# mrazomej/BarBay.jl

Measured on AMD Instinct MI355X. Metric: ELBO-grad steps/sec, 50k barcodes x 8 timepoints, higher is better.
Workload: dtype f64

## Files before the change

### barbay.jl_amd/csrc/bb_engine.hip

```cpp
#include "../../include/barbay_hip.h"
#include "bb_block.h"
#include "bb_persist.h"
#include "bb_resident.h"
#include "bb_stream.h"
#include "bb_inst.h"
#include "bb_hier.h"
#include "bb_ppc.h"

#include <algorithm>
#include <cmath>
#include <cstdarg>
#include <cstdio>
#include <cstdlib>
#include <cstring>
#include <ctime>
#include <string>
#include <type_traits>
#include <vector>

#ifndef BB_EMU
#include <dlfcn.h>
#endif

static thread_local char g_err[512] = "";
// ... 147 lines not shown
    const char* names[] = {"librccl.so.1", "librccl.so", "/opt/rocm/lib/librccl.so.1"};
    for (const char* n : names) {
        g_rccl.lib = dlopen(n, RTLD_NOW | RTLD_GLOBAL);
        if (g_rccl.lib) break;
    }
    if (!g_rccl.lib) return bb_fail(BB_ERR_COMM, "cannot load librccl: %s", dlerror());
    g_rccl.GetUniqueId = (int (*)(bb_ncclUniqueId*))dlsym(g_rccl.lib, "ncclGetUniqueId");
    g_rccl.CommInitRank = (int (*)(bb_ncclComm_t*, int, bb_ncclUniqueId, int))dlsym(g_rccl.lib, "ncclCommInitRank");
    g_rccl.AllReduce = (int (*)(const void*, void*, size_t, int, int, bb_ncclComm_t, hipStream_t))dlsym(g_rccl.lib, "ncclAllReduce");
    g_rccl.CommDestroy = (int (*)(bb_ncclComm_t))dlsym(g_rccl.lib, "ncclCommDestroy");
    g_rccl.GetErrorString = (const char* (*)(int))dlsym(g_rccl.lib, "ncclGetErrorString");
    if (!g_rccl.GetUniqueId || !g_rccl.CommInitRank || !g_rccl.AllReduce || !g_rccl.CommDestroy)
        return bb_fail(BB_ERR_COMM, "librccl lacks a required symbol");
    return 0;
}
#endif

#ifdef BB_EMU
struct DevGuard { explicit DevGuard(int) {} };
#else
struct DevGuard {
    int prev = -1, dev;
    explicit DevGuard(int d) : dev(d) { if (hipGetDevice(&prev) != hipSuccess) prev = -1; if (prev != dev) (void)hipSetDevice(dev); }
    ~DevGuard() { if (prev >= 0 && prev != dev) (void)hipSetDevice(prev); }
    DevGuard(const DevGuard&) = delete;
    DevGuard& operator=(const DevGuard&) = delete;
};
#endif
#define BB_ENTER(h) DevGuard bb_dev_guard_((h)->o.device)

struct BBTuning {
    bool no_hist_pack, no_host_tables, no_res, no_persist, no_stream, force_stream, any_parity, force_allreduce, p2p_self;
    bool no_graph, graph_collective, no_regroup, no_reorder, nb_set, lead_set;
    int nb, res_nb, ng, lead, nthr, row_l2;
};

static BBTuning read_tuning() {
    auto set = [](const char* n) { return getenv(n) != nullptr; };
    auto num = [](const char* n, int unset) { const char* v = getenv(n); return v ? atoi(v) : unset; };
    auto on = [&](const char* n) { return num(n, 0) > 0; };
    BBTuning t{};
    t.no_hist_pack = on("BB_NO_HIST_PACK");
    t.no_host_tables = on("BB_NO_HOST_TABLES");
    t.no_res = on("BB_NO_RES");
    t.no_persist = on("BB_NO_PERSIST");
    t.no_stream = on("BB_NO_STREAM");
    t.force_stream = on("BB_TUNE_STREAM");
    t.any_parity = on("BB_TUNE_AP");
    t.force_allreduce = on("BB_FORCE_ALLREDUCE");
    t.p2p_self = on("BB_P2P_SELF");
    t.no_graph = set("BB_NO_GRAPH");
    t.graph_collective = set("BB_GRAPH_COLLECTIVE");
    t.no_regroup = set("BB_NO_REGROUP");
    t.no_reorder = set("BB_NO_REORDER");
    t.nb_set = set("BB_TUNE_NB");
    t.nb = num("BB_TUNE_NB", 0);
    t.res_nb = num("BB_TUNE_RES_NB", 0);
    t.ng = num("BB_TUNE_NG", 0);
    t.lead_set = set("BB_TUNE_LEAD");
    t.lead = num("BB_TUNE_LEAD", 65);
    if (t.lead < 10 || t.lead > 100) t.lead = 100;
    t.nthr = num("BB_TUNE_NTHR", 0) >= 64 ? num("BB_TUNE_NTHR", 0) / 64 * 64 : 0;
    t.row_l2 = num("BB_TUNE_ROW_L2", 1) == 0 ? 0 : 1;
    return t;
}

enum { IMPL_TWO_KERNEL = 0, IMPL_PERSIST = 1, IMPL_RES = 2, IMPL_STREAM = 3 };
struct LaunchPlan {
    int impl = IMPL_TWO_KERNEL;
    int P = 0;
    int NB = 0, NBL = 0, nblk = 0;
    int ng = 8, pf = 0;
    bool ms = false;
    const void* fn = nullptr;
    std::string name;
    const char* why = nullptr;
};

struct bb_handle {
    DevModel M{};
    DevState S{};
    bb_advi_opts o{};
    std::vector<bb_block_range> blocks;
    std::vector<void*> owned;
    long long dev_bytes = 0;
    int NB = 0, nthr = 0, nblk = 0, ngeno_blk = 0;
    int tile_cap = 0;
    size_t lds_doubles = 0;
    size_t lds_doubles_p0 = 0;
    size_t lds_doubles_p = 0;
    long long b_lo = 0, b_hi = 0;
    int cus = 256;
    int g_lo = 0, g_hi = 0;
    std::vector<int> geno_ptr_h;
    long long* d_tile_b = nullptr;
// ... 561 lines not shown
    bb_handle* h = E.h;
    const RunArgs& A = E.A;
    BRSt<PP>* st = (BRSt<PP>*)E.st.data();
    auto cxof = [&](int b) { return BBCtx{h->nthr, b, E.lds.data() + (size_t)b * (h->lds_doubles_p + 64), nullptr}; };
    const BRLay& Y = h->Yh;
    const int NS = A.S < 1 ? 1 : A.S;
    const bool MSrun = NS > 1 || A.elbo_every > 0;
    const unsigned long long step = (unsigned long long)(h->step + it / NS);
    const int smp = (int)(it % NS);
    const bool last = smp == NS - 1;
    const unsigned long long xc = MSrun ? step * (unsigned long long)NS + (unsigned long long)smp : step;
    const int buf = (int)(xc & 1);
    const bool want_el = MSrun && A.elbo_every > 0 && step % (unsigned long long)A.elbo_every == 0;
    const int ring = A.elbo_every > 0 ? (int)((step / (unsigned long long)A.elbo_every) % BB_ELBO_RING) : 0;
    const bool xg = h->p2p_on;
    const BBSlot wslot = bb_slot_of(A, step);
    for (int b = 0; b < (phase == 2 ? bbp_groups(A) : h->plan.nblk); ++b) {
        BBCtx cx = cxof(b);
        BRSt<PP>* sb = st + (size_t)b * h->nthr;
        if (phase == 0) {
            br_prologue<KIND, PP, AP>(cx, h->M, h->S, A, Y, h->plan.NB, sb);
            br_draw_ahead<KIND, PP, AP>(cx, A, Y, sb, (unsigned long long)h->step);
        } else if (phase == 1) {
            if (MSrun) br_sample<KIND, PP, true>(cx, h->M, h->S, A, Y, sb, buf, wslot.slot, last, want_el);
            else br_sample<KIND, PP, false>(cx, h->M, h->S, A, Y, sb, buf, wslot.slot);
            const unsigned epoch = A.xepoch0 + (unsigned)(xc + 1);
            if (MSrun) br_moments<KIND, PP, true>(cx, h->M, h->S, Y, sb, buf, epoch, want_el);
            else br_moments<KIND, PP, false>(cx, h->M, h->S, Y, sb, buf, epoch);
            br_xchg_publish<KIND, PP, AP>(cx, h->M, h->S, A, Y, sb, xc, wslot.slot, last ? step + 1 : step, last ? 0u : (unsigned)(smp + 1), last);
        } else if (phase == 2) {
            if (xg) br_xchg_lead<true>(cx, h->M, h->S, A, Y, xc, &E.ok);
            else br_xchg_lead<false>(cx, h->M, h->S, A, Y, xc, &E.ok);
        } else if (phase == 3) {
            if (xg && MSrun) br_xchg_consume<KIND, PP, true, true>(cx, h->M, h->S, A, Y, sb, xc, &E.ok, want_el, ring, smp);
            else if (xg) br_xchg_consume<KIND, PP, true, false>(cx, h->M, h->S, A, Y, sb, xc, &E.ok);
            else if (MSrun) br_xchg_consume<KIND, PP, false, true>(cx, h->M, h->S, A, Y, sb, xc, &E.ok, want_el, ring, smp);
            else br_xchg_consume<KIND, PP, false, false>(cx, h->M, h->S, A, Y, sb, xc, &E.ok);
            if (MSrun) br_update<KIND, PP, 0, AP, true>(cx, h->M, h->S, A, Y, sb, wslot, buf, h->plan.NB, smp, NS);
            else if (!AP && uniform_T(h->M) == 8) br_update<KIND, PP, 8, false>(cx, h->M, h->S, A, Y, sb, wslot, buf, h->plan.NB);
            else if (!AP && uniform_T(h->M) == 6) br_update<KIND, PP, 6, false>(cx, h->M, h->S, A, Y, sb, wslot, buf, h->plan.NB);
            else br_update<KIND, PP, 0, AP>(cx, h->M, h->S, A, Y, sb, wslot, buf, h->plan.NB);
        } else {
            br_epilogue<KIND, PP, AP>(cx, h->S, sb, (unsigned long long)(h->step + nsteps), E.ok == 0);
        }
    }
}

template <int KIND, int TT, bool MS>
static void emu_stream_phase(EmuPersist& E, int phase, long long it, long long nsteps) {
    bb_handle* h = E.h;
    const RunArgs& A = E.A;
    BSG* gs = (BSG*)E.st.data();
    auto cxof = [&](int b) { return BBCtx{h->nthr, b, E.lds.data() + (size_t)b * (h->lds_doubles_p + 64), nullptr}; };
    const BRLay& Y = h->Yh;
    const int NS = MS ? (A.S < 1 ? 1 : A.S) : 1;
    const unsigned long long step = (unsigned long long)(h->step + it / NS);
    const int smp = (int)(it % NS);
    const unsigned long long xc = step * (unsigned long long)NS + (unsigned long long)smp;
    auto rec = [&](unsigned long long st_) { return MS && A.elbo_every > 0 && st_ % (unsigned long long)A.elbo_every == 0; };
    const bool want_el = rec(step);
    const int ring = A.elbo_every > 0 ? (int)((step / (unsigned long long)A.elbo_every) % BB_ELBO_RING) : 0;
    const BSMs ms = MS ? bs_ms_of(A, step, smp, NS, want_el, rec(step + 1)) : bs_ms_plain((unsigned)step);
    BRSt<1>* nost = nullptr;
    for (int b = 0; b < (phase == 2 ? bbp_groups(A) : h->plan.nblk); ++b) {
        BBCtx cx = cxof(b);
        BSG* gb = gs + (size_t)b * h->nthr;
        int* bad_any = (int*)(cx.lds + Y.L.misc) + 3;
        if (phase == 0) {
            br_tile_setup<KIND>(cx, h->M, h->S, A, Y, h->plan.NB, KIND <= 2 ? h->nthr / 16 : h->nthr / 64);
            *bad_any = 0;
// ... 577 lines not shown
    free(h->hstatus);
#else
    if (h->hstatus) (void)hipHostFree(h->hstatus);
#endif
    for (void* p : h->owned) dfree(p);
    if (h->eps_buf) dfree(h->eps_buf);
    if (h->dbg_buf) dfree(h->dbg_buf);
    if (h->ppc_buf) dfree(h->ppc_buf);
#ifndef BB_EMU
    if (h->stream) (void)hipStreamDestroy(h->stream);
#endif
    delete h;
}

extern "C" int64_t bb_num_latents(const bb_handle* h) { return h ? h->M.D : 0; }

extern "C" int bb_get_layout(const bb_handle* h, bb_block_range* blocks, int32_t* n) {
    if (!h || !blocks || !n) return bb_fail(BB_ERR_INVALID, "null argument");
    *n = (int32_t)h->blocks.size();
    for (size_t i = 0; i < h->blocks.size(); ++i) blocks[i] = h->blocks[i];
    return BB_OK;
}

static RunArgs make_args(const bb_handle* h, long long step, int sample, int S, bool apply, bool with_elbo) {
    RunArgs A;
    memset(&A, 0, sizeof A);
    A.b_lo = h->b_lo;
    A.b_hi = h->b_hi;
    A.rank = h->o.rank;
    A.world = h->o.world_size;
    A.xepoch0 = h->epoch0;
    A.spin_limit = 1u << 23;
    A.row_l2 = h->tune.row_l2;
    A.nblk = h->nblk;
    A.nblk_alloc = h->tile_cap - 8;
    A.ng = 8;
    A.par = (int)(step & 1);
    A.sample = sample;
    A.S = S;
    A.first_sample = sample == 0;
    A.last_sample = sample == S - 1;
    A.apply = apply ? 1 : 0;
    A.with_elbo = with_elbo ? 1 : 0;
    A.count_globals = h->o.rank == 0;
    A.opt = h->o.optimizer;
    A.W = h->o.window;
    A.resum_every = h->o.resum_every;
    A.elbo_every = h->o.elbo_every;
    A.eta = h->o.eta;
    A.tau = h->o.tau;
    A.pre = h->o.pre;
    A.post = h->o.post;
    A.seed = h->o.seed;
    A.elbo_const = h->elbo_const;
    if (h->use_reduce()) { A.red = h->S.totals; A.nred = 1; }
    else { A.red = h->S.partials; A.nred = h->nblk; }
    return A;
}

#ifdef BB_EMU
#define LAUNCH_CHECK() 0
#else
static int launch_check() {
    hipError_t e = hipGetLastError();
    if (e != hipSuccess) return bb_fail(BB_ERR_DEVICE, "kernel launch: %s", hipGetErrorString(e));
    return 0;
// ... 1257 lines not shown
```

### barbay.jl_amd/csrc/bb_persist.h

```cpp
#pragma once
#include "bb_block.h"
#include <string.h>

template <int KIND>
BB_DEV BBLds bbp_layout(const BBCtx& cx, const DevModel& M, int NB) {
    if (cx.lay) return *(const BBLds*)cx.lay;
    return bb_lds_layout(M.R, M.E, KIND, M.Ttot, M.nt1, M.K, NB, cx.nthr, 1);
}

template <int P>
struct BBPst {
    bb_d2 mu[P], om[P], am[P], ao[P];
    bb_d2 a[P], h[P];
    bb_d2 hm[P], ho[P];
    long long i0[P];
    int meta[P];
    bb_f4 lo[P];
};

#ifdef BB_EMU
#define BB_PSTATE(stv, tid) ((stv)[tid])
#else
#define BB_PSTATE(stv, tid) ((stv)[0])
#endif
// ... 398 lines not shown
        BB_SYNC(cx);
        BB_PASS(cx, tid) {
            if (tid < KK) {
                double s = lds[L.red + tid];
                for (int c = 1; c < chunks; ++c) s += lds[L.red + c * KKP + tid];
                if (XG) { for (int r = 0; r < A.world; ++r) bb_gran_st<true>(S.xgr[r] + bbx_slot(A, par, A.rank, g) * KK + tid, s, epoch); }
                else bb_gran_st(S.gxrow + ((long long)par * NG + g) * KK + tid, s, epoch);
            }
        }
        BB_SYNC(cx);
        BB_STAMP(cx, S, 18);
        return;
    }
    BB_PASS(cx, tid) {
        if (tid < KKP) {
            const bool act = tid < KK;
            const int k = act ? tid : KK - 1;
            double s = 0.0;
            for (int m0 = 0; m0 < members; m0 += 8) {
                double v[8];
                const int n = members - m0 < 8 ? members - m0 : 8;
                if (!bb_gran_poll8(S.grow + (long long)g * KS, (unsigned)(m0 * NG * KS + k), (unsigned)(NG * KS), n, epoch, act, S.gbar + 1, A.spin_limit, v)) *ok = 0;
#pragma unroll
                for (int i = 0; i < 8; ++i) s += v[i];
            }
            if (XG) {
                if (act) for (int r = 0; r < A.world; ++r) bb_gran_st<true>(S.xgr[r] + bbx_slot(A, par, A.rank, g) * KK + k, s, epoch);
            } else if (act) bb_gran_st(S.gxrow + ((long long)par * NG + g) * KK + k, s, epoch);
        }
    }
    BB_STAMP(cx, S, 18);
}

BB_DEV void bbp_consume_tg(BBCtx& cx, const DevModel& M, const DevState& S, const RunArgs& A, const BBLds& L, int par, unsigned epoch, int* ok) {
    double* lds = cx.lds;
    const int KK = M.K + 2 * M.nt1, NG = bbp_groups(A);
    const int KKP = (KK + 63) & ~63, NQ = (NG + 7) >> 3;
    double s0 = 0.0;
    BB_PASS(cx, tid) {
        const int q = (tid >= KKP ? 1 : 0) + (tid >= 2 * KKP ? 1 : 0) + (tid >= 3 * KKP ? 1 : 0) + (tid >= 4 * KKP ? 1 : 0), kk = tid - q * KKP;
        if (q < NQ) {
            const bool act = kk < KK;
            const int k = act ? kk : KK - 1, g0 = 8 * q;
            double v[8];
            const int n = NG - g0 < 8 ? NG - g0 : 8;
            if (!bb_gran_poll8(S.gxrow + (long long)par * NG * KK, (unsigned)(g0 * KK + k), (unsigned)KK, n, epoch, act, S.gbar + 1, A.spin_limit, v)) *ok = 0;
            double s = 0.0;
#pragma unroll
            for (int i = 0; i < 8; ++i) s += v[i];
            if (q > 0) { if (act) lds[L.red + (q - 1) * KKP + kk] = s; }
            else {
#ifdef BB_EMU
                if (act) lds[L.red + 3 * KKP + kk] = s;
#else
                s0 = s;
#endif
            }
        }
    }
    BB_STAMP(cx, S, 1);
    BB_SYNC(cx);
    BB_PASS(cx, tid) {
        if (tid < KK) {
#ifdef BB_EMU
            s0 = lds[L.red + 3 * KKP + tid];
#endif
            double s = s0;
            for (int q = 1; q < NQ; ++q) s += lds[L.red + (q - 1) * KKP + tid];
            if (tid < M.K) bb_put_total(M, L, lds, tid, s);
            else lds[L.zgl + (tid - M.K)] = s;
        }
    }
    if (!(KK <= 64 && M.Ttot <= 64)) BB_SYNC(cx);
}

BB_DEV void bbp_consume_tgx(BBCtx& cx, const DevModel& M, const DevState& S, const RunArgs& A, const BBLds& L, int par, unsigned epoch, int* ok) {
    double* lds = cx.lds;
    const int KK = M.K + 2 * M.nt1, KKP = (KK + 63) & ~63, chunks = A.world;
    int NQ = cx.nthr / KKP;
    if (NQ > chunks) NQ = chunks;
    if (NQ < 1) NQ = 1;
    const bb_gran* in = S.xgr[A.rank] + (long long)par * A.world * 8 * KK;
    BB_PASS(cx, tid) {
        int q = 0;
        for (int t = KKP; t <= tid && q < NQ; t += KKP) ++q;
        const int kk = tid - q * KKP;
        if (q < NQ) {
            const bool act = kk < KK;
            const int k = act ? kk : KK - 1;
            for (int c = q; c < chunks; c += NQ) {
                double v[8];
                if (!bb_gran_poll8<true>(in, (unsigned)(c * 8 * KK + k), (unsigned)KK, 8, epoch, act, S.gbar + 1, A.spin_limit, v)) *ok = 0;
                double s = 0.0;
#pragma unroll
// ... 313 lines not shown
```

### barbay.jl_amd/csrc/bb_resident.h

```cpp
#pragma once
#include "bb_persist.h"

#define BR_NCV 12
#if defined(BB_EMU) || defined(BR_NO_FENCE)
#define BR_SCHED_FENCE() ((void)0)
#else
#define BR_SCHED_FENCE() __builtin_amdgcn_sched_barrier(0)
#endif
#define BR_MAXT 16

struct BRSeg { long long lo, hi; int tbeg, span, blk, kind, ldsoff, r, lpb, T; double pm, iv; const double* mean_e; const double* iv_e; long long blo; int rstride, pad; };
#define BR_SEG_DOUBLES 12

struct BRLay {
    BBLds L;
    int zl, NBT;
    int zr0[BB_MAX_REP];
    int zlw, stw;
    int st[6], SU, nst;
    int eps;
    int hbuf;
    int racc;
    int racc_r[BB_MAX_REP], rw[BB_MAX_REP];
    int rowmap;
// ... 124 lines not shown
        Y.hbuf = o;    o += 4 * P * NT;
    } else {
        Y.hbuf = Y.racc;
        Y.eps = Y.hbuf + 4 * P * NT;
        busy = 6 * P * NT;
        o += racc_total > busy ? racc_total : busy;
    }
    { const int nch = xg_rows / 8 > 5 ? xg_rows / 8 : 5;
      L.red = o;     o += 2 * 128 + nch * ((KK + 63) & ~63) + 16; }
    (void)lmax;
    L.total = Y.total = (o + 1) & ~1;
    return Y;
}

template <int P>
struct BRSt {
    bb_d2 mu[P], om[P], am[P], ao[P];
    bb_d2 a[P], h[P];
    bb_d2 z[P];
    bb_d2 lam[P];
    long long i0[P];
    int meta[P];
    int zoff[P];
    int uo[P][3];
    int pt[P];
    int rb[P];
    int thoff[P];
    unsigned cnt[P][2];
    bb_f4 lo[P];
    bb_d2 gp[P];
    bb_d2 gm[P], go[P];
    double el;
};

enum { BRM_A0 = 1 << 4, BRM_A1 = 1 << 5, BRM_VALID = 1 << 6, BRM_MUT = 1 << 7, BRM_PREV = 1 << 8, BRM_NEXT = 1 << 9 };

template <bool AP> BB_DEV bool br_pair_aligned(long long i0) { return !AP || !(i0 & 1); }
template <bool AP> BB_DEV bb_d2 br_load_pair(const double* base, long long i0, bool a0, bool a1) {
    if (a0 && a1 && br_pair_aligned<AP>(i0)) return *(const bb_d2*)(base + i0);
    return bb_d2{a0 ? base[i0] : 0.0, a1 ? base[i0 + 1] : 0.0};
}
template <bool AP> BB_DEV void br_store_pair_stream(double* base, long long i0, bool a0, bool a1, bb_d2 v) {
#ifndef BB_EMU
    if (a0 && a1 && br_pair_aligned<AP>(i0)) {
        typedef double bb_v2d __attribute__((ext_vector_type(2)));
        bb_v2d w = {v.x, v.y};
        __builtin_nontemporal_store(w, (bb_v2d*)(base + i0));
        return;
    }
    if (a0) __builtin_nontemporal_store(v.x, base + i0);
    if (a1) __builtin_nontemporal_store(v.y, base + i0 + 1);
#else
    if (a0 && a1 && br_pair_aligned<AP>(i0)) { *(bb_d2*)(base + i0) = v; return; }
    if (a0) base[i0] = v.x;
    if (a1) base[i0 + 1] = v.y;
#endif
}
template <bool AP> BB_DEV void br_store_pair(double* base, long long i0, bool a0, bool a1, bb_d2 v) {
    if (a0 && a1 && br_pair_aligned<AP>(i0)) { *(bb_d2*)(base + i0) = v; return; }
    if (a0) base[i0] = v.x;
    if (a1) base[i0 + 1] = v.y;
}

BB_HD BBTile br_tile(const DevModel& M, const RunArgs& A, int block, int NB) {
    if (A.nbl <= 0) return bb_tile(M, A, block, NB);
    const int nlead = bbp_groups(A);
// ... 152 lines not shown
    st.meta[k] = meta;
}

BB_HD void br_table_row(const DevModel& M, const BRLay& Y, int j, int* rm2, int* tmapj) {
    int code = 0, col = 0;
    for (int r = 0; r < M.R; ++r) {
        const int T = M.T[r], q0 = j - M.kq[r];
        if (q0 < 0 || q0 >= 6 * T - 5) continue;
        int tt, q;
        if (q0 < T) { tt = q0; q = 0; } else { tt = (q0 - T) / 5; q = 1 + (q0 - T) - 5 * tt; }
        code = Y.lpb[r] | (1 << 24);
        col = Y.racc_r[r] + ((tt & 1) * 6 + q) * (Y.rw[r] + 4) + (tt >> 1);
    }
    rm2[0] = code;
    rm2[1] = col;
    int tj = -1;
    for (int r = 0; r < M.R; ++r) { const int tt = j - M.kq[r]; if (tt >= 0 && tt < M.T[r]) tj = M.tcum[r] + tt; }
    *tmapj = tj;
}
BB_HD void br_table_time(const DevModel& M, const BBLds& L, int j, int* ft) {
    int r = 0;
    while (r + 1 < M.R && j >= M.tcum[r + 1]) ++r;
    const int tt = j - M.tcum[r], T = M.T[r];
    ft[0] = tt < T - 1 ? L.wk + M.kq[r] + T + 5 * tt : -1;
    ft[1] = M.off_t[r] + tt;
    ft[2] = tt > 0 ? 1 : 0;
    ft[3] = 0;
}
BB_HD void br_table_rep(const DevModel& M, const BRLay& Y, int r, int* rt) {
    rt[0] = M.tcum[r]; rt[1] = Y.zr0[r]; rt[2] = M.T[r];
    rt[3] = M.cnt_off[r] < (1ll << 31) ? (int)M.cnt_off[r] : -1;
}

template <int KIND>
BB_DEV void br_tile_setup(BBCtx& cx, const DevModel& M, const DevState& S, const RunArgs& A, const BRLay& Y, int NB, int ncol_or_neg) {
    double* lds = cx.lds;
    const BBLds& L = Y.L;
    const BBTile t = KIND == 2 ? br_tile_geno(M, S, cx.block, NB) : br_tile(M, A, cx.block, NB);
    const int g0 = KIND == 2 ? S.tile_g[cx.block] : 0, g1 = KIND == 2 ? S.tile_g[cx.block + 1] : 0;
    BRSeg* sg = (BRSeg*)(lds + Y.seg);
    int* li = (int*)(lds + L.misc);
    const int KK = M.K + 2 * M.nt1;
    BB_PASS(cx, tid) {
        if (S.segtab) {
            const double* src = S.segtab + (long long)cx.block * S.segtab_stride;
            const int nd = S.segtab_stride - 1;
            for (int i = tid; i < nd; i += cx.nthr) lds[Y.seg + i] = src[i];
            if (tid == 0) li[0] = ((const int*)(src + nd))[0];
        } else if (tid == 0) li[0] = br_build_segs<KIND>(sg, M, Y, t, cx.block == 0, g0, g1);
        if (tid == 0) { li[1] = bb_get_word(S.gbar + 1) == 0u ? 1 : 0; li[2] = ncol_or_neg < 0 ? t.nbt : ncol_or_neg; }
        if (tid == 0) {
            const int xcc = br_xcc_id(), NG = bbp_groups(A);
            li[4] = A.row_l2 ? 0 : -1; li[5] = xcc; li[6] = (int)A.launch_tag; li[7] = NG;
            S.xsel[cx.block] = li[4];
            if (cx.block < NG) bb_set_word64(S.xtab + cx.block, ((unsigned long long)A.launch_tag << 32) | (unsigned)xcc);
        }
        for (int k = tid; k < KK; k += cx.nthr) lds[L.wk + k] = 0.0;
        for (int i = tid; i < Y.zlw * Y.NBT; i += cx.nthr) lds[Y.zl + i] = 0.0;
        for (int i = tid; i < Y.nst * Y.stw; i += cx.nthr) lds[Y.st[0] + i] = 0.0;
        if (tid <= M.Ttot) { lds[L.cc + tid] = 0.0; lds[L.wbar + tid] = 0.0; lds[L.Dt + tid] = 0.0; }
        if (tid < M.Ttot) ((int*)(lds + Y.envt))[tid] = (KIND == 1 || KIND == 4) ? M.env_idx[tid] : 0;
        if (S.ldstab) { for (int i = tid; i < 4 * M.R; i += cx.nthr) ((int*)(lds + Y.rtab))[i] = S.ldstab[3 * M.K + 4 * M.Ttot + i]; }
        else for (int rr = tid; rr < M.R; rr += cx.nthr) br_table_rep(M, Y, rr, (int*)(lds + Y.rtab) + 4 * rr);
        if (KIND == 2) {
            int* gx = (int*)(lds + Y.gix);
            for (int j = tid; j < t.nmt; j += cx.nthr) gx[j] = M.geno_idx[t.m0 + j] - g0;
            for (int j = tid; j < g1 - g0 && j < Y.SU; j += cx.nthr) {
                const int g = g0 + j, n = M.geno_ptr[g + 1] - M.geno_ptr[g];
                gx[Y.SU + j] = (n > 0 ? (int)(M.geno_mem[M.geno_ptr[g]] - t.m0) : 0) | (n << 16);
            }
        }
    }
    BB_STAMP_RT(cx, S, 7);
    BB_SYNC(cx);
    BB_STAMP_RT(cx, S, 8);
    int* rm = (int*)(lds + Y.rowmap);
    if (S.ldstab) {
        const int K = M.K, Tt = M.Ttot, R = M.R;
        BB_PASS(cx, tid) {
            for (int i = tid; i < 2 * K; i += cx.nthr) rm[i] = S.ldstab[i];
            for (int i = tid; i < K; i += cx.nthr) ((int*)(lds + L.tmap))[i] = S.ldstab[2 * K + i];
            for (int i = tid; i < 4 * Tt; i += cx.nthr) ((int*)(lds + Y.ftab))[i] = S.ldstab[3 * K + i];
        }
    } else {
        BB_PASS(cx, tid) {
            for (int j = tid; j < M.K; j += cx.nthr) br_table_row(M, Y, j, rm + 2 * j, (int*)(lds + L.tmap) + j);
            for (int j = tid; j < M.Ttot; j += cx.nthr) br_table_time(M, L, j, (int*)(lds + Y.ftab) + 4 * j);
        }
    }
    BB_STAMP_RT(cx, S, 9);
}

template <int KIND, int P, bool AP = false>
BB_DEV void br_prologue(BBCtx& cx, const DevModel& M, const DevState& S, const RunArgs& A, const BRLay& Y, int NB, BRSt<P>* stv) {
    double* lds = cx.lds;
    const BBLds& L = Y.L;
    const BBTile t = KIND == 2 ? br_tile_geno(M, S, cx.block, NB) : br_tile(M, A, cx.block, NB);
    const int g0 = KIND == 2 ? S.tile_g[cx.block] : 0, g1 = KIND == 2 ? S.tile_g[cx.block + 1] : 0;
    const BRSeg* sg = (const BRSeg*)(lds + Y.seg);
    const int* li = (const int*)(lds + L.misc);
    br_tile_setup<KIND>(cx, M, S, A, Y, NB, -1);
    BB_PASS(cx, tid) {
        const int nseg = li[0];
        BRSt<P>& st = BB_PSTATE(stv, tid);
#pragma unroll
        for (int k = 0; k < P; ++k) {
            br_desc<KIND, P, AP>(M, Y, t, sg, nseg, g0, g1, tid + k * cx.nthr, st, k, lds);
            const long long i0 = st.i0[k];
            const int meta = st.meta[k];
            const bool a0 = meta & BRM_A0, a1 = meta & BRM_A1;
            st.mu[k] = br_load_pair<AP>(S.mu, i0, a0, a1);
            st.om[k] = br_load_pair<AP>(S.om, i0, a0, a1);
            st.am[k] = br_load_pair<AP>(S.acc_mu, i0, a0, a1);
            st.ao[k] = br_load_pair<AP>(S.acc_om, i0, a0, a1);
            st.lo[k] = bb_load_lo(S, i0, a0, a1);
            st.a[k] = st.h[k] = st.z[k] = st.lam[k] = st.gp[k] = bb_d2{0.0, 0.0};
        }
    }
    BB_STAMP_RT(cx, S, 10);
    BB_SYNC(cx);
}

template <int P> struct BRIdx { long long i0[P]; int meta[P]; };

template <int P, bool MAYODD>
#ifdef BB_EMU
static inline
#else
__device__ __attribute__((noinline))
#endif
void br_draw_call(bb_d2* eps, int nthr, int tid, unsigned long long seed, unsigned step, unsigned stream,
                  long long i0a, long long i0b, long long i0c, long long i0d, int ma, int mb, int mc, int md) {
    BRIdx<P> ix;
    { const long long i0v[4] = {i0a, i0b, i0c, i0d}; const int mv[4] = {ma, mb, mc, md};
#pragma unroll
      for (int k = 0; k < P; ++k) { ix.i0[k] = i0v[k]; ix.meta[k] = mv[k]; } }
#pragma unroll
    for (int k = 0; k < P; ++k) {
        if (!(ix.meta[k] & BRM_VALID)) continue;
        const bool odd = MAYODD && (ix.i0[k] & 1);
        double e0 = 0.0, e1 = 0.0;
#pragma nounroll
        for (int rep = 0; rep < (odd ? 2 : 1); ++rep) {
            double a, b;
            bb_normal_pair(seed, (unsigned long long)(ix.i0[k] >> 1) + (unsigned long long)rep, step, stream, &a, &b);
            if (rep == 0) { e0 = odd ? b : a; e1 = b; }
            else e1 = a;
        }
        eps[k * nthr + tid] = bb_d2{e0, e1};
    }
}

template <int KIND, int P, bool AP = false>
// ... 173 lines not shown
            const int code = rm[2 * j], lpb = code & 255;
            const double* col = lds + rm[2 * j + 1];
            double s = 0.0;
#ifdef BB_EMU
            if (c == 0 && (code >> 24)) for (int e = 0; e < nbt; ++e) s += col[e * lpb];
#else
            if (code >> 24) for (int e = c; e < nbt; e += 16) s += col[e * lpb];
            s = br_row16_sum(s);
#endif
            if (c == 0) lds[Y.L.wk + j] = s;
        }
    }
    BB_SYNC(cx);
    int* li = (int*)(lds + Y.L.misc);
    BB_PASS(cx, tid) {
        if (li[4] > 0) { for (int j = tid; j < KK; j += cx.nthr) bb_gran_st_l2(S.grow + (long long)cx.block * KS + j, lds[Y.L.wk + j], epoch); }
        else for (int j = tid; j < KK; j += cx.nthr) bb_gran_st(S.grow + (long long)cx.block * KS + j, lds[Y.L.wk + j], epoch);
        if (tid == 0 && li[4] == 0) {
            int g = cx.block;
            while (g >= li[7]) g -= li[7];
            const unsigned long long v = bb_get_word64(S.xtab + g);
            if ((unsigned)(v >> 32) == (unsigned)li[6]) { li[4] = (int)(unsigned)v == li[5] ? 1 : -1; S.xsel[cx.block] = li[4]; }
        }
    }
    BB_STAMP(cx, S, 24);
    BB_STAMP_RT(cx, S, 29);
}

template <int KIND, int P, int TT> BB_DEV void br_theta_pre(BBCtx& cx, const DevModel& M, const BRLay& Y, BRSt<P>* stv, int buf);
template <int KIND, int P, bool MS = false>
BB_DEV void br_moments(BBCtx& cx, const DevModel& M, const DevState& S, const BRLay& Y, BRSt<P>* stv, int buf, unsigned epoch, bool want_el = false) {
    double* lds = cx.lds;
    if (KIND == 2) br_theta_pre<KIND, P, 0>(cx, M, Y, stv, buf);
    if (MS && want_el) {
        BB_PASS(cx, tid) {
            BRSt<P>& st = BB_PSTATE(stv, tid);
#ifdef BB_EMU
            (void)st;
#else
            double e = br_row16_sum(st.el);
            const int lo = __double2loint(e), hi = __double2hiint(e);
            double w = 0.0;
#pragma unroll
            for (int r = 0; r < 4; ++r) w += __hiloint2double(__builtin_amdgcn_readlane(hi, 16 * r), __builtin_amdgcn_readlane(lo, 16 * r));
            if ((tid & 63) == 0) lds[Y.L.part + (tid >> 6)] = w;
#endif
        }
    }
    BB_PASS(cx, tid) {
        BRSt<P>& st = BB_PSTATE(stv, tid);
#pragma unroll
        for (int k = 0; k < P; ++k) {
            const int meta = st.meta[k];
            if ((meta & 15) != SK_L) continue;
            double cv[BR_NCV];
#pragma unroll
            for (int q = 0; q < BR_NCV; ++q) cv[q] = 0.0;
            if (meta & BRM_VALID) {
            const double* zb = lds + Y.zl + buf * Y.NBT + st.zoff[k];
            const bool hn = meta & BRM_NEXT, mut = meta & BRM_MUT;
            const double z0 = st.z[k].x, z1 = st.z[k].y;
            const double zn = hn ? zb[2] : z1;
            double dm = z1 - z0, dn = zn - z1;
            cv[0] += st.lam[k].x;
            cv[6] += st.lam[k].y;
            if (mut) {
                double sm, sn, wm, wn;
                br_unit_sw<KIND>(lds, Y, buf, st.uo[k][1], KIND >= 2 ? st.thoff[k] : 0, &sm, &wm);
                if (KIND == 1 || KIND == 4) br_unit_sw<KIND>(lds, Y, buf, st.uo[k][2], KIND >= 3 ? st.thoff[k] : 0, &sn, &wn);
                else { sn = sm; wn = wm; }
                dm -= sm; dn -= sn;
                cv[1] += wm; cv[2] += wm * dm; cv[3] += wm * dm * dm;
                if (hn) { cv[7] += wn; cv[8] += wn * dn; cv[9] += wn * dn * dn; }
            } else {
                cv[4] += dm; cv[5] += dm * dm;
                if (hn) { cv[10] += dn; cv[11] += dn * dn; }
            }
            }
            {
                const BRSeg* sgk = (const BRSeg*)(lds + Y.seg) + (meta >> 12);
                const int stride = sgk->rstride;
#pragma unroll
                for (int q = 0; q < BR_NCV; ++q) lds[st.rb[k] + q * stride] = cv[q];
            }
        }
    }
    BB_SYNC(cx);
    br_row_publish<P, MS>(cx, M, S, Y, stv, epoch, want_el);
}

template <int P, bool HD>
BB_DEV void br_prefetch_slot(BBCtx& cx, const DevModel& M, const DevState& S, const RunArgs& A, const BRLay& Y, BRSt<P>* stv, int slot) {
    if (A.opt != 0) return;
    BB_PASS(cx, tid) {
        BRSt<P>& st = BB_PSTATE(stv, tid);
#pragma unroll
        for (int k = 0; k < P; ++k) {
            if (!(st.meta[k] & BRM_VALID)) continue;
#pragma unroll
            for (int which = 0; which < 2; ++which) {
                const double* src = S.hist + ((long long)slot * 2 + which) * M.Dh + (st.i0[k] - BR_HDELTA(HD, cx.lds, Y, st.meta[k]));
                bb_d2* dst = (bb_d2*)(cx.lds + Y.hbuf) + (k * 2 + which) * cx.nthr;
#ifdef BB_EMU
                dst[tid] = bb_d2{src[0], src[1]};
#else
                __builtin_amdgcn_global_load_lds((const __attribute__((address_space(1))) void*)src,
                                                 (__attribute__((address_space(3))) void*)(dst + (tid & ~63)), 16, 0, 0);
#endif
            }
        }
    }
}

template <int KIND, bool MS = false>
BB_DEV void br_finish(BBCtx& cx, const DevModel& M, const DevState& S, const BRLay& Y, const RunArgs* Ap = nullptr, bool want_el = false, int ring = 0, int smp = 0) {
    double* lds = cx.lds;
// ... 360 lines not shown
        for (int k = 0; k < P; ++k) {
            const int meta = st.meta[k];
            if (!(meta & BRM_VALID)) continue;
            const bool a0 = meta & BRM_A0, a1 = meta & BRM_A1;
            br_store_pair<AP>(S.mu, st.i0[k], a0, a1, st.mu[k]);
            br_store_pair<AP>(S.om, st.i0[k], a0, a1, st.om[k]);
            br_store_pair<AP>(S.acc_mu, st.i0[k], a0, a1, st.am[k]);
            br_store_pair<AP>(S.acc_om, st.i0[k], a0, a1, st.ao[k]);
            bb_store_lo(S, st.i0[k], a0, a1, st.lo[k]);
            const double chk = (a0 ? st.mu[k].x + st.om[k].x : 0.0) + (a1 ? st.mu[k].y + st.om[k].y : 0.0);
            bad = bad || !(chk - chk == 0.0);
        }
        if (bad) S.hstatus[1] = 1u;
        if (timed_out && tid == 0) S.hstatus[0] = 1u;
        if (cx.block == 0 && tid == 0) { S.ctr[0] = step_end; S.ctr[1] = step_end; }
    }
    BB_SYNC(cx);
}

template <int KIND, int P, bool AP = false, bool HD = false>
BB_DEV void br_xchg_publish(BBCtx& cx, const DevModel& M, const DevState& S, const RunArgs& A, const BRLay& Y, BRSt<P>* stv, unsigned long long xc, int slot,
                            unsigned long long next_step, unsigned next_stream = 0u, bool prefetch = true) {
    if (A.pf == 0 && prefetch) br_prefetch_slot<P, HD>(cx, M, S, A, Y, stv, slot);
    br_grad_pre<KIND, P, AP>(cx, Y, stv, (int)(xc & 1));
    br_theta_sum<KIND, P>(cx, M, Y, stv);
    if (KIND == 3) br_theta_pre<KIND, P, 0>(cx, M, Y, stv, (int)(xc & 1));
    br_draw_ahead<KIND, P, AP>(cx, A, Y, stv, next_step, next_stream);
}
template <bool XG>
BB_DEV void br_xchg_lead(BBCtx& cx, const DevModel& M, const DevState& S, const RunArgs& A, const BRLay& Y, unsigned long long xc, int* ok_slot) {
    const unsigned epoch = A.xepoch0 + (unsigned)(xc + 1);
    if (cx.block < bbp_groups(A)) bbp_leader_reduce_tg<XG>(cx, M, S, A, Y.L, (int)(xc & 1), epoch, ok_slot);
}
template <int KIND, int P, bool XG, bool MS = false>
BB_DEV void br_xchg_consume(BBCtx& cx, const DevModel& M, const DevState& S, const RunArgs& A, const BRLay& Y, BRSt<P>* stv,
                            unsigned long long xc, int* ok_slot, bool want_el = false, int ring = 0, int smp = 0) {
    const unsigned epoch = A.xepoch0 + (unsigned)(xc + 1);
    if (XG) bbp_consume_tgx(cx, M, S, A, Y.L, (int)(xc & 1), epoch, ok_slot);
    else bbp_consume_tg(cx, M, S, A, Y.L, (int)(xc & 1), epoch, ok_slot);
    br_finish<KIND, MS>(cx, M, S, Y, &A, want_el, ring, smp);
}

#ifndef BB_EMU
template <int KIND, int P, int NT, bool XG = false, int TT = 0, bool AP = false, bool MS = false>
__global__ void __launch_bounds__(NT) k_res(const DevModel* __restrict__ Mp, const DevState* __restrict__ Sp, const BRLay* __restrict__ Yp,
                                            RunArgs A, int NB, int nsteps) {
    const DevModel& M = *Mp;
    const DevState& S = *Sp;
    const BRLay& Y = *Yp;
    extern __shared__ __attribute__((aligned(16))) double br_smem[];
    BBCtx cx{(int)blockDim.x, (int)blockIdx.x, br_smem, nullptr};
    BRSt<P> st;
    int* ok_slot = (int*)(br_smem + Yp->L.misc) + 1;
    const unsigned long long c0 = S.ctr[0], c1 = S.ctr[1];
    unsigned long long step0 = c0 > c1 ? c0 : c1;
    step0 = ((unsigned long long)(unsigned)__builtin_amdgcn_readfirstlane((int)(step0 >> 32)) << 32) | (unsigned)__builtin_amdgcn_readfirstlane((int)step0);
    BB_STAMP_RT(cx, S, 2);
    br_prologue<KIND, P, AP>(cx, M, S, A, Y, NB, &st);
    BB_STAMP_RT(cx, S, 3);
    const bool dead = *ok_slot == 0;
    int done = 0;
    if (!dead) {
        br_draw_ahead<KIND, P, AP>(cx, A, Y, &st, step0);
        BB_STAMP_RT(cx, S, 4);
        BBSlotCtr sc = bb_slot_init(A, step0);
        const int NS = MS ? A.S : 1;
        int ec = (MS && A.elbo_every > 0) ? bb_uniform((int)(step0 % (unsigned long long)A.elbo_every)) : 1;
        int ring = (MS && A.elbo_every > 0) ? bb_uniform((int)(((step0 + (unsigned long long)A.elbo_every - 1ull) / (unsigned long long)A.elbo_every) % BB_ELBO_RING)) : 0;
        for (; done < nsteps; ++done, bb_slot_next(A, sc)) {
            const unsigned long long step = step0 + (unsigned long long)done;
            const BBSlot wslot = bb_slot_now(A, sc);
            const bool want_el = MS && A.elbo_every > 0 && ec == 0;
            bool stop = false;
            for (int smp = 0; smp < NS; ++smp) {
                const unsigned long long xc = MS ? step * (unsigned long long)NS + (unsigned long long)smp : step;
                const int buf = (int)(xc & 1);
                const bool last = smp == NS - 1;
                if (P > 1 || KIND >= 2) {
#pragma unroll
                    for (int k = 0; k < P; ++k) asm volatile("" : "+v"(st.meta[k]));
                }
                br_sample<KIND, P, MS, XG>(cx, M, S, A, Y, &st, buf, wslot.slot, last, want_el);
                br_moments<KIND, P, MS>(cx, M, S, Y, &st, buf, A.xepoch0 + (unsigned)(xc + 1), want_el);
                br_xchg_publish<KIND, P, AP, XG>(cx, M, S, A, Y, &st, xc, wslot.slot, last ? step + 1 : step, last ? 0u : (unsigned)(smp + 1), last);
                br_xchg_lead<XG>(cx, M, S, A, Y, xc, ok_slot);
                br_xchg_consume<KIND, P, XG, MS>(cx, M, S, A, Y, &st, xc, ok_slot, want_el, ring, smp);
                if (*ok_slot == 0) { stop = true; break; }
                br_update<KIND, P, TT, AP, MS, XG>(cx, M, S, A, Y, &st, wslot, buf, NB, smp, NS);
            }
            if (stop) break;
            if (MS && A.elbo_every > 0) {
                if (ec == 0) ring = ring + 1 == BB_ELBO_RING ? 0 : ring + 1;
                ec = ec + 1 == A.elbo_every ? 0 : ec + 1;
            }
        }
    }
    BB_STAMP_RT(cx, S, 5);
    asm volatile("s_waitcnt vmcnt(0)" ::: "memory");
    br_epilogue<KIND, P, AP>(cx, S, &st, step0 + (unsigned long long)done, dead || *ok_slot == 0);
    BB_STAMP_RT(cx, S, 6);
}
#endif
```

### barbay.jl_amd/csrc/bb_types.h

```cpp
#pragma once
#include <stdint.h>

#define BB_MAX_REP 16

enum BBBlockKind {
    BK_SPOP = 0,
    BK_LSPOP = 1,
    BK_S = 2,
    BK_TT = 3,
    BK_LT = 4,
    BK_LS = 5,
    BK_L = 6,
    BK_COUNT = 7
};

#define BB_NQ 6

struct DevPrior {
    double mean, inv_var;
    const double* mean_e;
    const double* inv_var_e;
};

struct DevModel {
// ... 60 lines not shown
    const long long *tile_b;
    const int *tile_g;
    unsigned long long *stamps;
    double *xout[BB_MAX_WORLD];
    unsigned *xout_rdy[BB_MAX_WORLD];
    struct bb_gran *xgr[BB_MAX_WORLD];
};

#define BB_ELBO_RING 4096

struct RunArgs {
    long long b_lo, b_hi;
    int rank, world;
    unsigned xepoch0;
    unsigned spin_limit;
    unsigned launch_tag;
    int row_l2;
    int nblk;
    int nblk_alloc;
    int ng;
    int pf;
    int nbl;
    int par;
    int sample, S;
    int first_sample, last_sample;
    int apply;
    int with_elbo;
    int count_globals;
    int opt, W, resum_every, elbo_every;
    double eta, tau, pre, post;
    unsigned long long seed;
    const double* red;
    int nred;
    double elbo_const;
};
```

Before: 72190.

## Skip dead moment classes in resident path and elide a barrier in own-group consume

After: 72400 (median of 2 runs). Within noise of the previous version (+0.3%).

```diff
diff --git a/barbay.jl_amd/csrc/bb_engine.hip b/barbay.jl_amd/csrc/bb_engine.hip
--- a/barbay.jl_amd/csrc/bb_engine.hip
+++ b/barbay.jl_amd/csrc/bb_engine.hip
@@ -203,7 +203,7 @@
 struct BBTuning {
     bool no_hist_pack, no_host_tables, no_res, no_persist, no_stream, force_stream, any_parity, force_allreduce, p2p_self;
     bool no_graph, graph_collective, no_regroup, no_reorder, nb_set, lead_set;
-    int nb, res_nb, ng, lead, nthr, row_l2;
+    int nb, res_nb, ng, lead, nthr, row_l2, res_generic;
 };
 
 static BBTuning read_tuning() {
@@ -232,6 +232,7 @@
     t.lead = num("BB_TUNE_LEAD", 65);
     if (t.lead < 10 || t.lead > 100) t.lead = 100;
     t.nthr = num("BB_TUNE_NTHR", 0) >= 64 ? num("BB_TUNE_NTHR", 0) / 64 * 64 : 0;
+    t.res_generic = on("BB_TUNE_RES_GENERIC") ? 1 : 0;
     t.row_l2 = num("BB_TUNE_ROW_L2", 1) == 0 ? 0 : 1;
     return t;
 }
@@ -859,10 +860,10 @@
             if (xg) br_xchg_lead<true>(cx, h->M, h->S, A, Y, xc, &E.ok);
             else br_xchg_lead<false>(cx, h->M, h->S, A, Y, xc, &E.ok);
         } else if (phase == 3) {
-            if (xg && MSrun) br_xchg_consume<KIND, PP, true, true>(cx, h->M, h->S, A, Y, sb, xc, &E.ok, want_el, ring, smp);
-            else if (xg) br_xchg_consume<KIND, PP, true, false>(cx, h->M, h->S, A, Y, sb, xc, &E.ok);
-            else if (MSrun) br_xchg_consume<KIND, PP, false, true>(cx, h->M, h->S, A, Y, sb, xc, &E.ok, want_el, ring, smp);
-            else br_xchg_consume<KIND, PP, false, false>(cx, h->M, h->S, A, Y, sb, xc, &E.ok);
+            if (xg && MSrun) br_xchg_consume<KIND, PP, true, true, true>(cx, h->M, h->S, A, Y, sb, xc, &E.ok, want_el, ring, smp);
+            else if (xg) br_xchg_consume<KIND, PP, true, false, true>(cx, h->M, h->S, A, Y, sb, xc, &E.ok);
+            else if (MSrun) br_xchg_consume<KIND, PP, false, true, true>(cx, h->M, h->S, A, Y, sb, xc, &E.ok, want_el, ring, smp);
+            else br_xchg_consume<KIND, PP, false, false, true>(cx, h->M, h->S, A, Y, sb, xc, &E.ok);
             if (MSrun) br_update<KIND, PP, 0, AP, true>(cx, h->M, h->S, A, Y, sb, wslot, buf, h->plan.NB, smp, NS);
             else if (!AP && uniform_T(h->M) == 8) br_update<KIND, PP, 8, false>(cx, h->M, h->S, A, Y, sb, wslot, buf, h->plan.NB);
             else if (!AP && uniform_T(h->M) == 6) br_update<KIND, PP, 6, false>(cx, h->M, h->S, A, Y, sb, wslot, buf, h->plan.NB);
@@ -1506,6 +1507,7 @@
     A.xepoch0 = h->epoch0;
     A.spin_limit = 1u << 23;
     A.row_l2 = h->tune.row_l2;
+    A.res_generic = h->tune.res_generic;
     A.nblk = h->nblk;
     A.nblk_alloc = h->tile_cap - 8;
     A.ng = 8;
diff --git a/barbay.jl_amd/csrc/bb_persist.h b/barbay.jl_amd/csrc/bb_persist.h
--- a/barbay.jl_amd/csrc/bb_persist.h
+++ b/barbay.jl_amd/csrc/bb_persist.h
@@ -454,6 +454,7 @@
     BB_STAMP(cx, S, 18);
 }
 
+template <bool OWN = false>
 BB_DEV void bbp_consume_tg(BBCtx& cx, const DevModel& M, const DevState& S, const RunArgs& A, const BBLds& L, int par, unsigned epoch, int* ok) {
     double* lds = cx.lds;
     const int KK = M.K + 2 * M.nt1, NG = bbp_groups(A);
@@ -481,7 +482,7 @@
         }
     }
     BB_STAMP(cx, S, 1);
-    BB_SYNC(cx);
+    if (!(OWN && NQ == 1 && KK <= 64)) BB_SYNC(cx);
     BB_PASS(cx, tid) {
         if (tid < KK) {
 #ifdef BB_EMU
diff --git a/barbay.jl_amd/csrc/bb_resident.h b/barbay.jl_amd/csrc/bb_resident.h
--- a/barbay.jl_amd/csrc/bb_resident.h
+++ b/barbay.jl_amd/csrc/bb_resident.h
@@ -180,6 +180,9 @@
     bb_d2 gm[P], go[P];
     double el;
 };
+
+enum { BR_DEAD_M = 0x0e, BR_DEAD_N = 0x30 };
+BB_HD int br_dead_classes(const BBTile& t) { return (t.nmt == 0 ? BR_DEAD_M : 0) | (t.nshift == 0 ? BR_DEAD_N : 0); }
 
 enum { BRM_A0 = 1 << 4, BRM_A1 = 1 << 5, BRM_VALID = 1 << 6, BRM_MUT = 1 << 7, BRM_PREV = 1 << 8, BRM_NEXT = 1 << 9 };
 
@@ -398,7 +401,7 @@
     rt[3] = M.cnt_off[r] < (1ll << 31) ? (int)M.cnt_off[r] : -1;
 }
 
-template <int KIND>
+template <int KIND, bool DC = false>
 BB_DEV void br_tile_setup(BBCtx& cx, const DevModel& M, const DevState& S, const RunArgs& A, const BRLay& Y, int NB, int ncol_or_neg) {
     double* lds = cx.lds;
     const BBLds& L = Y.L;
@@ -415,6 +418,7 @@
             if (tid == 0) li[0] = ((const int*)(src + nd))[0];
         } else if (tid == 0) li[0] = br_build_segs<KIND>(sg, M, Y, t, cx.block == 0, g0, g1);
         if (tid == 0) { li[1] = bb_get_word(S.gbar + 1) == 0u ? 1 : 0; li[2] = ncol_or_neg < 0 ? t.nbt : ncol_or_neg; }
+        if (DC && tid == 0) li[8] = A.res_generic ? 0 : br_dead_classes(t);
         if (tid == 0) {
             const int xcc = br_xcc_id(), NG = bbp_groups(A);
             li[4] = A.row_l2 ? 0 : -1; li[5] = xcc; li[6] = (int)A.launch_tag; li[7] = NG;
@@ -465,7 +469,7 @@
     const int g0 = KIND == 2 ? S.tile_g[cx.block] : 0, g1 = KIND == 2 ? S.tile_g[cx.block + 1] : 0;
     const BRSeg* sg = (const BRSeg*)(lds + Y.seg);
     const int* li = (const int*)(lds + L.misc);
-    br_tile_setup<KIND>(cx, M, S, A, Y, NB, -1);
+    br_tile_setup<KIND, P == 1>(cx, M, S, A, Y, NB, -1);
     BB_PASS(cx, tid) {
         const int nseg = li[0];
         BRSt<P>& st = BB_PSTATE(stv, tid);
@@ -485,6 +489,18 @@
     }
     BB_STAMP_RT(cx, S, 10);
     BB_SYNC(cx);
+    const int dead = P == 1 ? li[8] : 0;
+    if (dead) {
+        int* rm = (int*)(lds + Y.rowmap);
+        BB_PASS(cx, tid) {
+            for (int j = tid; j < M.K; j += cx.nthr)
+                for (int r = 0; r < M.R; ++r) {
+                    const int T = M.T[r], q0 = j - M.kq[r];
+                    if (q0 < T || q0 >= 6 * T - 5) continue;
+                    if ((dead >> (1 + (q0 - T) % 5)) & 1) rm[2 * j] &= ~(1 << 24);
+                }
+        }
+    }
 }
 
 template <int P> struct BRIdx { long long i0[P]; int meta[P]; };
@@ -724,6 +740,7 @@
 BB_DEV void br_moments(BBCtx& cx, const DevModel& M, const DevState& S, const BRLay& Y, BRSt<P>* stv, int buf, unsigned epoch, bool want_el = false) {
     double* lds = cx.lds;
     if (KIND == 2) br_theta_pre<KIND, P, 0>(cx, M, Y, stv, buf);
+    const int dead = P == 1 ? bb_uniform(((const int*)(lds + Y.L.misc))[8]) : 0;
     if (MS && want_el) {
         BB_PASS(cx, tid) {
             BRSt<P>& st = BB_PSTATE(stv, tid);
@@ -772,8 +789,21 @@
             {
                 const BRSeg* sgk = (const BRSeg*)(lds + Y.seg) + (meta >> 12);
                 const int stride = sgk->rstride;
-#pragma unroll
-                for (int q = 0; q < BR_NCV; ++q) lds[st.rb[k] + q * stride] = cv[q];
+                if (P > 1) {
+#pragma unroll
+                    for (int q = 0; q < BR_NCV; ++q) lds[st.rb[k] + q * stride] = cv[q];
+                    continue;
+                }
+                lds[st.rb[k]] = cv[0];
+                lds[st.rb[k] + 6 * stride] = cv[6];
+                if (!(dead & BR_DEAD_M)) {
+#pragma unroll
+                    for (int q = 1; q < 4; ++q) { lds[st.rb[k] + q * stride] = cv[q]; lds[st.rb[k] + (q + 6) * stride] = cv[q + 6]; }
+                }
+                if (!(dead & BR_DEAD_N)) {
+#pragma unroll
+                    for (int q = 4; q < 6; ++q) { lds[st.rb[k] + q * stride] = cv[q]; lds[st.rb[k] + (q + 6) * stride] = cv[q + 6]; }
+                }
             }
         }
     }
@@ -1200,12 +1230,12 @@
     const unsigned epoch = A.xepoch0 + (unsigned)(xc + 1);
     if (cx.block < bbp_groups(A)) bbp_leader_reduce_tg<XG>(cx, M, S, A, Y.L, (int)(xc & 1), epoch, ok_slot);
 }
-template <int KIND, int P, bool XG, bool MS = false>
+template <int KIND, int P, bool XG, bool MS = false, bool OWN = false>
 BB_DEV void br_xchg_consume(BBCtx& cx, const DevModel& M, const DevState& S, const RunArgs& A, const BRLay& Y, BRSt<P>* stv,
                             unsigned long long xc, int* ok_slot, bool want_el = false, int ring = 0, int smp = 0) {
     const unsigned epoch = A.xepoch0 + (unsigned)(xc + 1);
     if (XG) bbp_consume_tgx(cx, M, S, A, Y.L, (int)(xc & 1), epoch, ok_slot);
-    else bbp_consume_tg(cx, M, S, A, Y.L, (int)(xc & 1), epoch, ok_slot);
+    else bbp_consume_tg<OWN>(cx, M, S, A, Y.L, (int)(xc & 1), epoch, ok_slot);
     br_finish<KIND, MS>(cx, M, S, Y, &A, want_el, ring, smp);
 }
 
@@ -1252,7 +1282,7 @@
                 br_moments<KIND, P, MS>(cx, M, S, Y, &st, buf, A.xepoch0 + (unsigned)(xc + 1), want_el);
                 br_xchg_publish<KIND, P, AP, XG>(cx, M, S, A, Y, &st, xc, wslot.slot, last ? step + 1 : step, last ? 0u : (unsigned)(smp + 1), last);
                 br_xchg_lead<XG>(cx, M, S, A, Y, xc, ok_slot);
-                br_xchg_consume<KIND, P, XG, MS>(cx, M, S, A, Y, &st, xc, ok_slot, want_el, ring, smp);
+                br_xchg_consume<KIND, P, XG, MS, true>(cx, M, S, A, Y, &st, xc, ok_slot, want_el, ring, smp);
                 if (*ok_slot == 0) { stop = true; break; }
                 br_update<KIND, P, TT, AP, MS, XG>(cx, M, S, A, Y, &st, wslot, buf, NB, smp, NS);
             }
diff --git a/barbay.jl_amd/csrc/bb_types.h b/barbay.jl_amd/csrc/bb_types.h
--- a/barbay.jl_amd/csrc/bb_types.h
+++ b/barbay.jl_amd/csrc/bb_types.h
@@ -116,5 +116,6 @@
     unsigned long long seed;
     const double* red;
     int nred;
+    int res_generic;
     double elbo_const;
 };
```
